# CliMA/LandHydrology.jl

Hardware: AMD Instinct MI355X
Metric: column-cell updates/sec (RHS evals) (higher is better)
Workload: dtype f64

## Files before the change

### landhydrology.jl_amd/csrc/lh_heat_implicit.hpp

```cpp
#pragma once
#include "lh_kernels_impl.hpp"

namespace lh {

template <typename M>
constexpr int heat_implicit_threads() {
    return M::uses_tables ? 512 : 256;
}

template <typename FT>
__device__ __forceinline__ FT heat_boundary_flux(const DevParams<FT>& P, const FaceState<FT>& fs, int face, int64_t col,
                                                 FT T_c) {
    FT fe, fw;
    boundary_fluxes_from<FT, MODEL_HEAT>(P, fs, face, col, T_c, FT(0), FT(0), fe, fw);
    return fe * P.inv_dz;
}

template <typename FT, typename M, bool PERCOL, bool TRBDF2>
__device__ __forceinline__ void heat_implicit_column(const M& mm, DevParams<FT> P, const HeatImplicitArgs<FT>& A,
                                                     int64_t col, FT& nf_acc) {
    const int n = P.nlev;
    const int64_t stride = P.stride;
    const int64_t top = int64_t(n - 1) * stride + col;
    const FT coef = A.coef;
// ... 121 lines not shown
            boundary_constants(kb, kt);
            {
                FT ay = A.al[col] * y[col], be = A.be[col];
                FT Flo = fb_n - Gb * ay;
                forward(kb, kt, [&](int i, int64_t idx) {
                    FT Fhi, ayu = FT(0), beu = FT(0);
                    if (i + 1 < n) {
                        const int64_t idu = idx + stride;
                        ayu = A.al[idu] * y[idu];
                        beu = A.be[idu];
                        Fhi = -A.ks[idx] * (((ayu - ay) + (beu - be)) * P.cg2);
                    } else {
                        Fhi = ft_n + Gt * ay;
                    }
                    const FT f = Flo - Fhi;
                    Flo = Fhi;
                    ay = ayu;
                    be = beu;
                    return y[idx] + coef * f;
                });
            }
            backward([&](int64_t idx, FT x) { z[idx] = (x - c_yn * y[idx]) * c_w2; });
            faces_at(vb1, vt1);
            boundary_constants(kb, kt);
            forward(kb, kt, [&](int, int64_t idx) { return z[idx]; });
            backward(store_y);
        }
    }
}

template <typename FT, typename M, bool PERCOL, bool TRBDF2>
__global__ void __launch_bounds__(heat_implicit_threads<M>())
heat_implicit_kernel(const DevParams<FT> P, const HeatImplicitArgs<FT> A) {
    __shared__ double s_tab[M::uses_tables ? MATH_TAB_DOUBLES : 2];
    const M mm(stage_math_tables<M>(P.math_tab, s_tab));
    const int64_t col = int64_t(blockIdx.x) * blockDim.x + threadIdx.x;
    if (col >= P.ncols) return;
    FT nf_acc = FT(0);
    heat_implicit_column<FT, M, PERCOL, TRBDF2>(mm, P, A, col, nf_acc);
    if (nf_acc != nf_acc) atomicOr(P.status, 1u);
}

template <typename FT>
void launch_heat_implicit(const DevParams<FT>& P, const HeatImplicitArgs<FT>& A, bool percol, bool trbdf2, int math,
                          hipStream_t s) {
    with_math<FT>(math == MATH_LIBM, [&](auto m) { with_bool(percol, [&](auto pc) { with_bool(trbdf2, [&](auto tr) {
        using M = typename decltype(m)::type;
        hipLaunchKernelGGL((heat_implicit_kernel<FT, M, decltype(pc)::value, decltype(tr)::value>),
                           grid_for(P.ncols, heat_implicit_threads<M>()), dim3(heat_implicit_threads<M>()), 0, s, P, A);
    }); }); });
}

#define LH_INSTANTIATE_HEAT_IMPLICIT(FT) \
    template void launch_heat_implicit<FT>(const DevParams<FT>&, const HeatImplicitArgs<FT>&, bool, bool, int, hipStream_t);

}
```

### landhydrology.jl_amd/csrc/lh_implicit.hpp

```cpp
#pragma once
#include "lh_kernels_impl.hpp"

namespace lh {


#define LH_IMPLICIT_DMAX_FRAC 0.5
#define LH_IMPLICIT_STALL 0.9
#define LH_TRBDF2_MAX_STEPS 100000
#define LH_TRBDF2_HMIN_FRAC 1e-10

template <typename FT, bool NOICE>
__device__ __forceinline__ void water_slopes(const ColC<FT>& c, FT vl, FT ti, FT npsi, float& dkr, float& dnpsi) {
    using MF = MathFast<float>;
    dkr = 0.0f;
    dnpsi = 0.0f;
    if (!(vl > c.theta_lim)) return;
    const float num = float(vl - c.theta_r);
    const float m = float(c.m), inv_m = float(c.inv_m);
    const float S = num * float(c.inv_por);
    float w = 0.0f;
    if (S < 1.0f) {
        const float t = MF::exp2(MF::log2(S) * inv_m);
        w = fmaxf(1.0f - t, 1e-7f);
        const float wm = MF::exp2(MF::log2(w) * m);
// ... 16 lines not shown

template <typename FT>
__device__ __forceinline__ FT boundary_flux_slope(const DevParams<FT>& P, const FaceState<FT>& fs, int face,
                                                  FT dK_c, FT dnpsi_c) {
    const int kh = face == FACE_BOTTOM ? P.bc_kind[FACE_BOTTOM][COMP_HYDROLOGY] : P.bc_kind[FACE_TOP][COMP_HYDROLOGY];
    const FT inv_dzb = FT(2) * P.inv_dz;
    if (kh == BC_FREE_DRAINAGE) return -dK_c;
    if (kh == BC_DIRICHLET) {
        return face == FACE_BOTTOM ? fs.K * dnpsi_c * inv_dzb : -fs.K * dnpsi_c * inv_dzb;
    }
    return FT(0);
}

template <typename M>
constexpr int implicit_threads() {
    return M::uses_tables ? 512 : 256;
}

template <typename M>
constexpr bool implicit_variant_exists(bool noice, bool vgf) { return M::is_production || (!noice && !vgf); }

template <typename FT, typename F>
inline void with_implicit_variant(const DevParams<FT>& P, bool percol, bool noice, int math, F&& f) {
    const bool libm = math == MATH_LIBM;
    const bool ni = noice && !libm;
    const bool vg = !libm && !(sizeof(FT) == 8 && P.vg_fast_all == 0);
    with_math<FT>(libm, [&](auto m) { with_bool(percol, [&](auto pc) { with_bool(ni, [&](auto i) { with_bool(vg, [&](auto v) {
        if constexpr (implicit_variant_exists<typename decltype(m)::type>(decltype(i)::value, decltype(v)::value)) f(m, pc, i, v);
    }); }); }); });
}

template <typename M>
__device__ __forceinline__ M implicit_math(const double* math_tab) {
    __shared__ double s_tab[M::uses_tables ? MATH_TAB_DOUBLES : 2];
    return M(stage_math_tables<M>(math_tab, s_tab));
}
__device__ __forceinline__ int64_t implicit_lane_column() { return int64_t(blockIdx.x) * blockDim.x + threadIdx.x; }

template <typename FT, typename M, bool PERCOL, bool NOICE>
struct ColumnSolve {
    static constexpr bool RELK = M::is_production;
    ColC<FT> c;
    FT Ksc, cgw, dmax, floor_r;
    __device__ __forceinline__ ColumnSolve(const M& mm, const DevParams<FT>& P, int64_t col) {
        c = make_colc<FT, M>(P, col, PERCOL);
        if (!NOICE) finish_colc<FT, M>(mm, c);
        Ksc = RELK ? c.Ksat : FT(1);
        cgw = RELK ? c.cgw : P.cg2;
        dmax = FT(LH_IMPLICIT_DMAX_FRAC) * (c.nu - c.theta_r);
        floor_r = c.theta_r;
    }
};

template <typename FT, typename M, bool PERCOL, bool NOICE, bool VGF, bool JAC, typename Row, bool STORE = false>
__device__ __forceinline__ void column_sweep_up(const M& mm, const DevParams<FT>& P,
                                                const ColumnSolve<FT, M, PERCOL, NOICE>& S, const FaceState<FT>& fsb,
                                                const FaceState<FT>& fst, int64_t col, const FT* y, const FT* ti,
                                                FT ti_b, FT coef, FT* cp, FT* dp, Row&& row, FT* sa = nullptr,
                                                FT* sden = nullptr) {
    constexpr bool RELK = ColumnSolve<FT, M, PERCOL, NOICE>::RELK;
    constexpr bool vgf = VGF && M::uses_tables;
    const ColC<FT>& c = S.c;
    const FT Ksc = S.Ksc, cgw = S.cgw;
    const int n = P.nlev;
    const int64_t stride = P.stride;
    const FT T = FT(288);
    auto closures = [&](FT v, FT tiv, FT& K, FT& np, FT& dK, FT& dn) {
// ... 394 lines not shown
```

### landhydrology.jl_amd/csrc/lh_kernels_impl.hpp

```cpp
#pragma once
#include "lh_closures.hpp"
#include "lh_launch.hpp"
#include "lh_dispatch.hpp"
#include "lh_atmos.hpp"
#include <type_traits>

namespace lh {

#ifndef LH_RHS_WAVES_PER_SIMD
#define LH_RHS_WAVES_PER_SIMD 8
#endif
#ifndef LH_RHS_F64_WAVES
#define LH_RHS_F64_WAVES 6
#endif

#ifndef LH_F32C_DT_WAVES
#define LH_F32C_DT_WAVES 5
#endif
#ifndef LH_F32C_DT_VGPRCONST
#define LH_F32C_DT_VGPRCONST 1
#endif
#ifndef LH_F32C_DT_WAVES_SGPR
#define LH_F32C_DT_WAVES_SGPR 8
#endif
// ... 74 lines not shown
    using V = typename Vec<FT, N>::type;
    V v;
    FT* e = reinterpret_cast<FT*>(&v);
#pragma unroll
    for (int j = 0; j < N; ++j) e[j] = in[j];
    if (NT) __builtin_nontemporal_store(v, reinterpret_cast<V*>(p));
    else *reinterpret_cast<V*>(p) = v;
}

template <typename FT, int N, bool NT>
__device__ __forceinline__ void bload(const FT* row, unsigned row_bytes, unsigned lane_byte, FT (&out)[N]) {
    static_assert(sizeof(FT) * N == 8, "one 8-byte access per lane");
    typedef unsigned u32x2 __attribute__((ext_vector_type(2)));
    __amdgpu_buffer_rsrc_t rs = __builtin_amdgcn_make_buffer_rsrc(const_cast<FT*>(row), 0, row_bytes, 0x00020000);
    u32x2 v = __builtin_amdgcn_raw_buffer_load_b64(rs, lane_byte, 0, NT ? 2 : 0);
    __builtin_memcpy(out, &v, 8);
}
template <typename FT, int N, bool NT>
__device__ __forceinline__ void bstore(FT* row, unsigned row_bytes, unsigned lane_byte, const FT (&in)[N]) {
    static_assert(sizeof(FT) * N == 8, "one 8-byte access per lane");
    typedef unsigned u32x2 __attribute__((ext_vector_type(2)));
    __amdgpu_buffer_rsrc_t rs = __builtin_amdgcn_make_buffer_rsrc(row, 0, row_bytes, 0x00020000);
    u32x2 v;
    __builtin_memcpy(&v, in, 8);
    __builtin_amdgcn_raw_buffer_store_b64(v, rs, lane_byte, 0, NT ? 2 : 0);
}

template <int CPL_, int PF_, bool NT_, bool SEG_>
struct KCfg {
    static constexpr int CPL = CPL_, PF = PF_;
    static constexpr bool NT = NT_, SEG = SEG_;
};

template <typename M>
__device__ __forceinline__ MathTables stage_math_tables(const double* gtab, double* lds) {
    MathTables t;
    t.log_tab = lds;
    t.exp_tab = lds + 2 * LOG_TAB_N;
    if (M::uses_tables) {
        for (int i = threadIdx.x; i < MATH_TAB_DOUBLES; i += blockDim.x) lds[i] = gtab[i];
        __syncthreads();
    }
    return t;
}

template <typename FT> struct Bits;
template <> struct Bits<double> { using type = unsigned long long; };
template <> struct Bits<float> { using type = unsigned int; };

__device__ __forceinline__ double fmax_ft(double a, double b) { return __builtin_fmax(a, b); }
__device__ __forceinline__ float fmax_ft(float a, float b) { return __builtin_fmaxf(a, b); }
__device__ __forceinline__ double fmin_ft(double a, double b) { return __builtin_fmin(a, b); }
__device__ __forceinline__ float fmin_ft(float a, float b) { return __builtin_fminf(a, b); }

__device__ __forceinline__ float max_nonneg(float a, float b) {
    return __builtin_bit_cast(float, __builtin_elementwise_max(__builtin_bit_cast(int, a), __builtin_bit_cast(int, b)));
}

__device__ __forceinline__ void wave_sync() {
    __builtin_amdgcn_fence(__ATOMIC_RELEASE, "wavefront");
    __builtin_amdgcn_wave_barrier();
    __builtin_amdgcn_fence(__ATOMIC_ACQUIRE, "wavefront");
}

template <typename FT>
__device__ __forceinline__ bool finite(FT x) {
    return x - x == FT(0);
}

template <typename M>
constexpr bool noice_exists(bool factors) { return M::is_production && !factors; }
template <typename M, int MODEL>
constexpr bool robust_vg_exists() { return M::uses_tables && MODEL != MODEL_HEAT; }
// ... 16 lines not shown
    constexpr bool WATER = (MODEL != MODEL_HEAT);
    constexpr bool HEAT = (MODEL != MODEL_RICHARDS);
    constexpr bool TEND_MODE = (MODE == 0 || MODE == 4);
    DevParams<FT> P = P0;
    if constexpr (heat_vgpr_constants<FT, MODEL, FACTORS, PERCOL, M, NOICE>() && TEND_MODE && (!FACTORS || PERCOL || MODE == 4)) {
        auto vr = [](FT& x) { asm volatile("" : "+v"(x)); };
        vr(P.rho_c_ds); vr(P.rhocp_l); vr(P.rhocp_i); vr(P.T_ref); vr(P.kappa_sat_unfrozen);
        vr(P.l2_kappa_sat_unfrozen); vr(P.l2_kappa_sat_frozen); vr(P.kersten_exp_unfrozen);
        vr(P.kersten_exp_frozen); vr(P.neg_b_log2e_sc);
        if (MODE != 4) {
            vr(P.rho_i); vr(P.LH_f0); vr(P.inv_dz); vr(P.half_inv_dz);
            if (FACTORS) { vr(P.gamma); vr(P.T_ref_visc); vr(P.Omega); }
        }
    }
#ifndef LH_F64_FACTORS_PARTIAL_PIN
#define LH_F64_FACTORS_PARTIAL_PIN 3
#endif
#ifndef LH_F64_FACTORS_PARTIAL_PIN_STAGES
#define LH_F64_FACTORS_PARTIAL_PIN_STAGES 0
#endif
    if constexpr (LH_F64_FACTORS_PARTIAL_PIN > 0 && heat_vgpr_constants<FT, MODEL, FACTORS, PERCOL, M, NOICE>() &&
                  (MODE == 0 || (LH_F64_FACTORS_PARTIAL_PIN_STAGES && MODE != 4)) &&
                  FACTORS && !PERCOL) {
        auto vr = [](FT& x) { asm volatile("" : "+v"(x)); };
        vr(P.rho_c_ds); vr(P.rhocp_l); vr(P.T_ref);
        if (LH_F64_FACTORS_PARTIAL_PIN >= 5) { vr(P.rhocp_i); vr(P.rho_i); }
        if (LH_F64_FACTORS_PARTIAL_PIN >= 8) { vr(P.LH_f0); vr(P.gamma); vr(P.Omega); }
    }
    constexpr int CPL = CFG::CPL, PF = CFG::PF;
    constexpr bool NT = CFG::NT;
    constexpr bool TEND = (MODE == 0 || MODE == 4);
    constexpr bool WANT_DT = (MODE == 4);
    const FT dt = (!TEND && dt_device) ? *dt_device : dt_value;
    __shared__ double s_tab[M::uses_tables ? MATH_TAB_DOUBLES : 2];
    extern __shared__ __align__(16) unsigned char s_dyn[];
    const int n = P.nlev;
    float* s_red = reinterpret_cast<float*>(s_dyn);
    if (WANT_DT) s_red[threadIdx.x] = 0.0f;
    __shared__ unsigned s_waves_done;
    if (WANT_DT && threadIdx.x == 0) s_waves_done = 0u;
    constexpr bool MAY_PROF = (MODEL == MODEL_HEAT) || (MODEL == MODEL_RICHARDS && FACTORS);
    FT* s_pf = reinterpret_cast<FT*>(s_dyn + (WANT_DT ? ((size_t(blockDim.x) * sizeof(float) + 15) & ~size_t(15)) : 0));
    const FT* pf_T = (MAY_PROF && MODEL == MODEL_RICHARDS) ? P.aux_prof[3] : nullptr;
    const FT* pf_vl = (MAY_PROF && MODEL == MODEL_HEAT) ? P.aux_prof[0] : nullptr;
    const FT* pf_ti = (MAY_PROF && MODEL == MODEL_HEAT) ? P.aux_prof[1] : nullptr;
    if constexpr (MAY_PROF) {
        for (int i = threadIdx.x; i < n; i += blockDim.x) {
            if (pf_T) s_pf[i] = pf_T[i];
            if (pf_vl) s_pf[i] = pf_vl[i];
            if (pf_ti) s_pf[n + i] = pf_ti[i];
        }
    }
    const M mm(stage_math_tables<M>(P.math_tab, s_tab));
    if (!M::uses_tables) __syncthreads();

    unsigned blk = blockIdx.x;
    if (P.xcd_remap) {
        const unsigned per = gridDim.x >> 3;
        if (blk < (per << 3)) blk = (blk & 7u) * per + (blk >> 3);
    }
    const int64_t col0 = (int64_t(blk) * blockDim.x + threadIdx.x) * CPL;
    if (col0 >= P.ncols) return;
    const int64_t stride = P.stride;
    constexpr bool SEG = CFG::SEG;
    const int i_lo = SEG ? int(blockIdx.y) * P.seg_len : 0;
    const int i_hi = SEG ? (i_lo + P.seg_len < n ? i_lo + P.seg_len : n) : n;
    const int i_first = (SEG && i_lo > 0) ? i_lo - 1 : 0;
    const int i_end = (SEG && i_hi < n) ? i_hi + 1 : n;
    const unsigned lane_byte = (unsigned)col0 * (unsigned)sizeof(FT);
    const unsigned row_bytes = (unsigned)(stride * (int64_t)sizeof(FT));
    constexpr bool BUF = (sizeof(FT) * CPL == 8);
    auto rload = [&](const FT* row, FT (&out)[CPL]) {
        if constexpr (BUF) bload<FT, CPL, NT>(row, row_bytes, lane_byte, out);
        else vload<FT, CPL, NT>(row + col0, out);
    };
    auto rstore = [&](FT* row, const FT (&in)[CPL]) {
        if constexpr (BUF) bstore<FT, CPL, NT>(row, row_bytes, lane_byte, in);
        else vstore<FT, CPL, NT>(row + col0, in);
    };

    const int64_t in0 = SEG ? stride * i_first : 0, out0 = SEG ? stride * i_lo : 0;
    constexpr bool FROM_K1 = (MODE == 5);
    const FT* r_vl = (MODEL == MODEL_HEAT ? AUX.v[0] : (FROM_K1 ? BASE.v[0] : IN.v[0])) + in0;
    const FT* r_ti = NOICE ? nullptr : (MODEL == MODEL_HEAT ? AUX.v[1] : (TEND ? IN.v[1] : BASE.v[1])) + in0;
    const FT* r_re = HEAT ? (FROM_K1 ? BASE.v[2] : IN.v[2]) + in0 : nullptr;
    const FT* r_k1v = (FROM_K1 && WATER) ? IN.v[0] + in0 : nullptr;
    const FT* r_k1e = (FROM_K1 && HEAT) ? IN.v[2] + in0 : nullptr;
    const bool need_Taux = (MODEL == MODEL_RICHARDS) && FACTORS && P.viscosity_kind;
    const FT* r_Ta = need_Taux ? AUX.v[3] + in0 : nullptr;
    const FT* b_vl = ((MODE == 2 || MODE == 3) && WATER) ? BASE.v[0] + out0 : nullptr;
    const FT* b_re = ((MODE == 2 || MODE == 3) && HEAT) ? BASE.v[2] + out0 : nullptr;
    FT* o_vl = WATER ? OUT.v[0] + out0 : nullptr;
    FT* o_re = HEAT ? OUT.v[2] + out0 : nullptr;

    ColC<FT> c[CPL];
    int64_t colj[CPL];
#pragma unroll
    for (int j = 0; j < CPL; ++j) {
        colj[j] = col0 + j < P.ncols ? col0 + j : P.ncols - 1;
        c[j] = make_colc<FT, M>(P, colj[j], PERCOL);
        if (WATER && !NOICE) finish_colc<FT, M>(mm, c[j]);
        if constexpr (M::uses_tables && WATER && !PERCOL && !HEAT) asm volatile("" : "+v"(c[j].e_log2_alpha));
    }
    if constexpr (f32_coupled_vgpr_constants<FT, MODEL, FACTORS, PERCOL, M, MODE>()) {
        auto vr = [](FT& x) { asm volatile("" : "+v"(x)); };
        ColC<FT>& q = c[0];
        vr(q.nu); vr(q.theta_lim); vr(q.theta_r); vr(q.inv_por); vr(q.e_inv_m); vr(q.e_m); vr(q.e_one);
        vr(q.e_inv_n); vr(q.e_log2_alpha); vr(q.Ksat); vr(q.inv_S_s); vr(q.inv_nu); vr(q.k_dry);
        if (!NOICE) vr(q.l2_por);
#pragma unroll
        for (int j = 1; j < CPL; ++j) c[j] = c[0];
    }

    constexpr bool vgf = VGF && M::uses_tables;
    constexpr bool RELK = M::is_production;
    const FT cgT = P.cg2;
    FT cgw[CPL], Ksc[CPL];
#pragma unroll
    for (int j = 0; j < CPL; ++j) {
        Ksc[j] = RELK ? c[j].Ksat : FT(1);
        cgw[j] = RELK ? c[j].cgw : cgT;
    }

    FT vl[CPL], ti[CPL], re[CPL], Ta[CPL];
    FT vl_n[PF][CPL], ti_n[PF][CPL], re_n[PF][CPL], Ta_n[PF][CPL];
    FT kv_n[PF][CPL], ke_n[PF][CPL];
    FT vl_p[CPL], re_p[CPL];
    FT yv[CPL], ye[CPL], yv_p[CPL], ye_p[CPL];
    FT K_p[CPL], psi_p[CPL], T_p[CPL], kap_p[CPL], E_p[CPL];
    FT Fw_lo[CPL], Fe_lo[CPL];
    FT nf_acc = FT(0);
    float dpsi_p[CPL], ircs_p[CPL], DmaxW[CPL], DmaxT[CPL];
    float DmaxWb[CPL];

#pragma unroll
    for (int j = 0; j < CPL; ++j) {
        K_p[j] = psi_p[j] = T_p[j] = kap_p[j] = E_p[j] = Fw_lo[j] = Fe_lo[j] = FT(0);
        vl_p[j] = re_p[j] = FT(0);
        yv[j] = ye[j] = yv_p[j] = ye_p[j] = FT(0);
        vl[j] = ti[j] = re[j] = FT(0);
        Ta[j] = FT(288);
        dpsi_p[j] = DmaxW[j] = DmaxWb[j] = DmaxT[j] = ircs_p[j] = 0.0f;
    }
    int lev_f = i_first;
    auto fetch = [&](int slot) {
        if (MAY_PROF && pf_vl) {
#pragma unroll
            for (int j = 0; j < CPL; ++j) vl_n[slot][j] = s_pf[lev_f];
        } else rload(r_vl, vl_n[slot]);
        if (!NOICE) {
            if (MAY_PROF && pf_ti) {
#pragma unroll
                for (int j = 0; j < CPL; ++j) ti_n[slot][j] = s_pf[n + lev_f];
            } else rload(r_ti, ti_n[slot]);
        }
        if (HEAT) rload(r_re, re_n[slot]);
        if (need_Taux) {
            if (MAY_PROF && pf_T) {
#pragma unroll
                for (int j = 0; j < CPL; ++j) Ta_n[slot][j] = s_pf[lev_f];
            } else rload(r_Ta, Ta_n[slot]);
        }
        ++lev_f;
        if (FROM_K1 && WATER) { rload(r_k1v, kv_n[slot]); r_k1v += stride; }
        if (FROM_K1 && HEAT) { rload(r_k1e, ke_n[slot]); r_k1e += stride; }
        r_vl += stride;
        if (!NOICE) r_ti += stride;
        if (HEAT) r_re += stride;
        if (need_Taux) r_Ta += stride;
    };
#pragma unroll
    for (int k = 0; k < PF; ++k) {
#pragma unroll
        for (int j = 0; j < CPL; ++j) {
            vl_n[k][j] = ti_n[k][j] = re_n[k][j] = kv_n[k][j] = ke_n[k][j] = FT(0);
            Ta_n[k][j] = FT(288);
        }
        if (i_first + k < i_end) fetch(k);
    }

    auto emit = [&](const FT (&Fw_hi)[CPL], const FT (&Fe_hi)[CPL], const FT (&u_vl)[CPL],
                    const FT (&u_re)[CPL], const FT (&y_vl)[CPL], const FT (&y_re)[CPL]) {
        FT dvl[CPL], dre[CPL];
#pragma unroll
        for (int j = 0; j < CPL; ++j) {
            dvl[j] = WATER ? Fw_lo[j] - Fw_hi[j] : FT(0);
            dre[j] = HEAT ? Fe_lo[j] - Fe_hi[j] : FT(0);
            if (CPL == 1 || col0 + j < P.ncols) {
                if (WATER) nf_acc = fma_ft(dvl[j], FT(0), nf_acc);
                if (HEAT) nf_acc = fma_ft(dre[j], FT(0), nf_acc);
            }
        }
        if (TEND) {
            if (WATER) rstore(o_vl, dvl);
            if (HEAT) rstore(o_re, dre);
        } else {
            auto stage = [&](const FT* brow, FT* orow, const FT (&u)[CPL], const FT (&k)[CPL], const FT (&yb)[CPL]) {
                FT b[CPL], r[CPL];
                if (MODE == 2 || MODE == 3) rload(brow, b);
#pragma unroll
                for (int j = 0; j < CPL; ++j) {
                    if (FROM_K1) b[j] = yb[j];
                    if (MODE == 1)
                        r[j] = u[j] + dt * k[j];
                    else if (MODE == 2 || MODE == 5)
                        r[j] = (FT(3) * b[j] + u[j] + dt * k[j]) * FT(0.25);
                    else {
                        const FT sum = b[j] + FT(2) * u[j] + FT(2) * dt * k[j];
                        const FT q = sum * FT(1.0 / 3.0);
                        r[j] = fma_ft(fma_ft(FT(-3), q, sum), FT(1.0 / 3.0), q);
                    }
// ... 4 lines not shown
            if (HEAT) stage(b_re, o_re, u_re, dre, y_re);
        }
        if (WATER) {
            o_vl += stride;
            if (MODE == 2 || MODE == 3) b_vl += stride;
        }
        if (HEAT) {
            o_re += stride;
            if (MODE == 2 || MODE == 3) b_re += stride;
        }
    };

#if LH_RHS_OUTER_UNROLL > 0
#pragma unroll RHS_OUTER_UNROLL
#endif
    for (int i0 = i_first; i0 < i_end; i0 += PF) {
#pragma unroll
      for (int k = 0; k < PF; ++k) {
        const int i = i0 + k;
        if (PF > 1 && i >= i_end) break;
#pragma unroll
        for (int j = 0; j < CPL; ++j) {
            vl[j] = vl_n[k][j];
            ti[j] = NOICE ? FT(0) : ti_n[k][j];
            re[j] = re_n[k][j];
            Ta[j] = Ta_n[k][j];
            if (FROM_K1) {
                yv[j] = vl[j];
                ye[j] = re[j];
                if (WATER) vl[j] = yv[j] + dt * kv_n[k][j];
                if (HEAT) re[j] = ye[j] + dt * ke_n[k][j];
            }
        }
        if (i + PF < i_end) fetch(k);
        FT K[CPL], psi[CPL], T[CPL], kap[CPL], E[CPL], rcs[CPL];
        float dpsi[CPL], ircs[CPL];
#pragma unroll
        for (int j = 0; j < CPL; ++j) {
            T[j] = Ta[j];
            kap[j] = FT(0);
            K[j] = psi[j] = E[j] = FT(0);
            dpsi[j] = ircs[j] = 0.0f;
            rcs[j] = FT(1);
            if (HEAT) {
                T[j] = temperature_closure<FT, M, NOICE>(mm, P, c[j], vl[j], ti[j], re[j], rcs[j]);
                kap[j] = kappa_closure<FT, M, NOICE>(mm, P, c[j], vl[j], ti[j]);
                if (WANT_DT) ircs[j] = float(mm.rcp(rcs[j]));
            }
            if (WATER) {
                water_closures<FT, M, FACTORS, true, WANT_DT, NOICE, RELK, HEAT, true>(mm, P, c[j], vl[j], ti[j], T[j], K[j],
                                                                                       psi[j], &dpsi[j], vgf);
                if (HEAT) E[j] = (P.rhocp_l * (T[j] - P.T_ref)) * K[j];
            }
            if (WANT_DT && i > i_first) {
                if (WATER) DmaxW[j] = max_nonneg(DmaxW[j], float(K_p[j] + K[j]) * max_nonneg(dpsi_p[j], dpsi[j]));
                if (HEAT) DmaxT[j] = max_nonneg(DmaxT[j], float(kap_p[j] + kap[j]) * max_nonneg(ircs_p[j], ircs[j]));
            }
        }
        if (i == 0) {
#pragma unroll
            for (int j = 0; j < CPL; ++j) {
                FT K_f = FT(0), kap_f = FT(0);
                const FT K_c = K[j] * Ksc[j];
                boundary_fluxes<FT, M, MODEL, FACTORS, NOICE>(mm, P, c[j], FACE_BOTTOM, colj[j], vl[j], ti[j],
                                                              T[j], K_c, -psi[j], Fe_lo[j], Fw_lo[j], &K_f, &kap_f, vgf);
                Fe_lo[j] = Fe_lo[j] * P.inv_dz;
                Fw_lo[j] = Fw_lo[j] * P.inv_dz;
// ... 1 lines not shown
                    DmaxW[j] = max_nonneg(DmaxW[j], 2.0f * float(K[j]) * dpsi[j]);
                    DmaxWb[j] = max_nonneg(DmaxWb[j], 4.0f * float(fmax_ft(K_f, K_f > FT(0) ? K_c : FT(0))) * dpsi[j]);
                    if (HEAT) {
                        DmaxT[j] = max_nonneg(DmaxT[j], 2.0f * float(kap[j]) * ircs[j]);
                        DmaxT[j] = max_nonneg(DmaxT[j], 4.0f * float(fmax_ft(kap_f, kap_f > FT(0) ? kap[j] : FT(0))) * ircs[j]);
                    }
                }
            }
        } else if (!SEG || i > i_first) {
            FT Fw[CPL], Fe[CPL];
#pragma unroll
            for (int j = 0; j < CPL; ++j) {
                Fw[j] = Fe[j] = FT(0);
                FT gh = FT(0);
                if (WATER) {
                    gh = head_difference(psi[j], psi_p[j], P.dz) * cgw[j];
                    Fw[j] = -(K_p[j] + K[j]) * gh;
                }
                if (HEAT) {
                    FT gT = (T[j] - T_p[j]) * cgT;
                    Fe[j] = -(kap_p[j] + kap[j]) * gT;
                    if (WATER) Fe[j] = Fe[j] - (E_p[j] + E[j]) * gh;
                }
            }
            if (!SEG || i > i_lo) emit(Fw, Fe, vl_p, re_p, yv_p, ye_p);
#pragma unroll
            for (int j = 0; j < CPL; ++j) {
                Fw_lo[j] = Fw[j];
                Fe_lo[j] = Fe[j];
            }
        }
#pragma unroll
        for (int j = 0; j < CPL; ++j) {
            vl_p[j] = vl[j];
            re_p[j] = re[j];
            if (FROM_K1) {
                yv_p[j] = yv[j];
                ye_p[j] = ye[j];
            }
            K_p[j] = K[j];
            psi_p[j] = psi[j];
            T_p[j] = T[j];
            kap_p[j] = kap[j];
            E_p[j] = E[j];
            if (WANT_DT) {
                dpsi_p[j] = dpsi[j];
                ircs_p[j] = ircs[j];
            }
        }
      }
    }
    if (!SEG || i_hi == n) {
        FT Fw[CPL], Fe[CPL];
#pragma unroll
        for (int j = 0; j < CPL; ++j) {
            FT K_f = FT(0), kap_f = FT(0);
            const FT K_c = K_p[j] * Ksc[j];
            boundary_fluxes<FT, M, MODEL, FACTORS, NOICE>(mm, P, c[j], FACE_TOP, colj[j], vl[j], ti[j], T_p[j],
                                                          K_c, -psi_p[j], Fe[j], Fw[j], &K_f, &kap_f, vgf);
            Fe[j] = Fe[j] * P.inv_dz;
            Fw[j] = Fw[j] * P.inv_dz;
            if (WANT_DT) {
                DmaxW[j] = max_nonneg(DmaxW[j], 2.0f * float(K_p[j]) * dpsi_p[j]);
                DmaxWb[j] = max_nonneg(DmaxWb[j], 4.0f * float(fmax_ft(K_f, K_f > FT(0) ? K_c : FT(0))) * dpsi_p[j]);
                if (HEAT) {
                    DmaxT[j] = max_nonneg(DmaxT[j], 2.0f * float(kap_p[j]) * ircs_p[j]);
                    DmaxT[j] = max_nonneg(DmaxT[j], 4.0f * float(fmax_ft(kap_f, kap_f > FT(0) ? kap_p[j] : FT(0))) * ircs_p[j]);
                }
            }
        }
        emit(Fw, Fe, vl_p, re_p, yv_p, ye_p);
    }
    if (nf_acc != nf_acc) atomicOr(P.status, 1u);
    if (WANT_DT) {
        using U = typename Bits<FT>::type;
        float dmax = 0.0f;
#pragma unroll
        for (int j = 0; j < CPL; ++j) {
// ... 18 lines not shown
            const unsigned nw = lanes_left >= int64_t(blockDim.x) ? nwaves : unsigned((lanes_left + 63) >> 6);
            if (atomicAdd(&s_waves_done, 1u) == nw - 1u) {
                for (unsigned w = 0; w < nwaves; ++w) dmax = max_nonneg(dmax, s_red[w << 6]);
                if (dmax > 0.0f) {
                    const FT best = (FT(2) * dt * P.dz * P.dz) / FT(dmax);
                    U b;
                    __builtin_memcpy(&b, &best, sizeof(FT));
                    U* word = reinterpret_cast<U*>(P.dt_out);
                    if (b < __atomic_load_n(word, __ATOMIC_RELAXED)) atomicMin(word, b);
                }
            }
        }
    }
}

constexpr int CS_FACE_WORDS = 8;
template <int MODEL> constexpr int cs_exchange_arrays() {
    return MODEL == MODEL_COUPLED ? 5 : 2;
}
template <int MODEL> constexpr int cs_flux_arrays() {
    return MODEL == MODEL_COUPLED ? 2 : 1;
}
static inline int cs_fetch_tiles(int model, bool noice, bool need_Taux) {
    if (model == MODEL_RICHARDS) return 1 + (noice ? 0 : 1) + (need_Taux ? 2 : 0);
    return 3;
}

template <typename FT, int MODEL, bool FACTORS, bool PERCOL, typename M, bool NOICE = false, bool VGF = true>
__global__ void __launch_bounds__(1024)
column_stepper_kernel(const DevParams<FT> P0, const Planes<FT> Y, const Planes<FT> AUX, const FT dt_value,
                      const FT* __restrict__ dt_device, const int64_t nsteps, const FT* __restrict__ bcv) {
    constexpr bool WATER = (MODEL != MODEL_HEAT);
    constexpr bool HEAT = (MODEL != MODEL_RICHARDS);
    __shared__ double s_tab[M::uses_tables ? MATH_TAB_DOUBLES : 2];
    extern __shared__ __align__(16) unsigned char s_dyn[];
    const int n = P0.nlev;
    const int tpc = (n + 63) & ~63;
    const int slot = int(threadIdx.x) / tpc;
    const int cpb = int(blockDim.x) / tpc;
    const FT dt = dt_device ? *dt_device : dt_value;
    constexpr int NARR = cs_exchange_arrays<MODEL>();
    FT* sK = reinterpret_cast<FT*>(s_dyn) + size_t(slot) * NARR * n;
    FT* sh = sK + n;
    FT* sT = WATER ? sh + n : sK;
    FT* sKap = sT + n;
    FT* sE = sKap + n;
    const M mm(stage_math_tables<M>(P0.math_tab, s_tab));
    if (!M::uses_tables) __syncthreads();
    DevParams<FT> P = P0;
    const int i = int(threadIdx.x) - slot * tpc;
    unsigned blk = blockIdx.x;
    if (P.xcd_remap) {
        const unsigned per = gridDim.x >> 3;
        if (blk < (per << 3)) blk = (blk & 7u) * per + (blk >> 3);
    }
    const int64_t col_raw = int64_t(blk) * cpb + slot;
    const bool cell = i < n && col_raw < P.ncols;
    const int ic = i < n ? i : n - 1;
    const int64_t col = col_raw < P.ncols ? col_raw : P.ncols - 1;
    ColC<FT> c = make_colc<FT, M>(P, col, PERCOL);
    if (WATER && !NOICE) finish_colc<FT, M>(mm, c);
    constexpr bool vgf = VGF && M::uses_tables;
    constexpr bool RELK = M::is_production;
    const FT cgT = P.cg2;
    const FT Ksc = RELK ? c.Ksat : FT(1);
    const FT cgw = RELK ? c.cgw : cgT;
    const bool need_Taux = (MODEL == MODEL_RICHARDS) && FACTORS && P.viscosity_kind;
// ... 125 lines not shown
        if (col_first + cs < P.ncols) {
            const int64_t g = int64_t(lev) * P.stride + col_first + cs;
            if (WATER) Y.v[0][g] = tiles[cs * n + lev];
            if (HEAT) Y.v[2][g] = tiles[tile_n + cs * n + lev];
        }
    }
    if (cell && nf_acc != nf_acc) atomicOr(P.status, 1u);
}

template <typename T>
__device__ __forceinline__ T wave_uniform(const T& x) {
    static_assert(sizeof(T) % 4 == 0, "32-bit words");
    uint32_t w[sizeof(T) / 4];
    __builtin_memcpy(w, &x, sizeof(T));
#pragma unroll
    for (size_t k = 0; k < sizeof(T) / 4; ++k) w[k] = __builtin_amdgcn_readfirstlane(w[k]);
    T r;
    __builtin_memcpy(&r, w, sizeof(T));
    return r;
}

template <typename FT, int MODEL, bool FACTORS, bool PERCOL, typename M, int CW, bool NOICE>
constexpr int cs_wave_min_waves() {
    if (!M::uses_tables || MODEL != MODEL_RICHARDS) return 4;
    if (CW == 1) return 6;
    return (NOICE && !FACTORS) ? 6 : 4;
}
template <typename FT, int MODEL, bool FACTORS, bool PERCOL, typename M, int CW, bool NOICE = false, bool VGF = true, bool BOUND = false>
__global__ void __launch_bounds__(1024, (cs_wave_min_waves<FT, MODEL, FACTORS, PERCOL, M, CW, NOICE>()))
column_stepper_wave_kernel(const DevParams<FT> P0, const Planes<FT> Y, const Planes<FT> AUX, const FT dt_value,
                           const FT* __restrict__ dt_device, const int64_t nsteps, const FT* __restrict__ bcv) {
    constexpr bool WATER = (MODEL != MODEL_HEAT);
    constexpr bool HEAT = (MODEL != MODEL_RICHARDS);
    __shared__ double s_tab[M::uses_tables ? MATH_TAB_DOUBLES : 2];
    extern __shared__ __align__(16) unsigned char s_dyn[];
    const int n = P0.nlev;
    const int slot = int(threadIdx.x) >> 6;
    const int l = int(threadIdx.x) & 63;
    const int cpb = int(blockDim.x) >> 6;
    const FT dt = dt_device ? *dt_device : dt_value;
    constexpr int NEX = cs_exchange_arrays<MODEL>();
    constexpr int NARR = NEX + cs_flux_arrays<MODEL>();
    constexpr size_t COLW = size_t(NARR) * 64 + CS_FACE_WORDS;
    FT* sK = reinterpret_cast<FT*>(s_dyn) + size_t(slot) * COLW;
    FT* sh = sK + 64;
    FT* sT = WATER ? sh + 64 : sK;
    FT* sKap = sT + 64;
    FT* sE = sKap + 64;
    FT* sFw = sK + size_t(NEX) * 64;
    FT* sFe = WATER ? sFw + 64 : sFw;
    FT* sFace = sK + size_t(NARR) * 64;
    const M mm(stage_math_tables<M>(P0.math_tab, s_tab));
    if (!M::uses_tables) __syncthreads();
    DevParams<FT> P = P0;
    unsigned blk = blockIdx.x;
    if (P.xcd_remap) {
        const unsigned per = gridDim.x >> 3;
        if (blk < (per << 3)) blk = (blk & 7u) * per + (blk >> 3);
    }
    const int64_t col_raw = int64_t(blk) * cpb + slot;
    const int64_t col = col_raw < P.ncols ? col_raw : P.ncols - 1;
    ColC<FT> c = make_colc<FT, M>(P, col, PERCOL);
    if (WATER && !NOICE) finish_colc<FT, M>(mm, c);
    if constexpr (PERCOL) c = wave_uniform(c);
    constexpr bool vgf = VGF && M::uses_tables;
    constexpr bool RELK = M::is_production;
    const FT cgT = P.cg2;
// ... 267 lines not shown
                U b;
                __builtin_memcpy(&b, &best, sizeof(FT));
                U* word = reinterpret_cast<U*>(P.dt_out);
                if (b < __atomic_load_n(word, __ATOMIC_RELAXED)) atomicMin(word, b);
            }
        }
    }
    __syncthreads();
#pragma unroll
    for (int q = 0; q < CW; ++q) {
        const int i = CW * l + q;
        if (i < n) {
            if (WATER) tiles[slot * n + i] = y_vl[q];
            if (HEAT) tiles[tile_n + slot * n + i] = y_re[q];
        }
    }
    __syncthreads();
    for (int e = threadIdx.x; e < tile_n; e += blockDim.x) {
        const int lev = e / cpb, cs = e - lev * cpb;
        if (col_first + cs < P.ncols) {
            const int64_t g = int64_t(lev) * P.stride + col_first + cs;
            if (WATER) Y.v[0][g] = tiles[cs * n + lev];
            if (HEAT) Y.v[2][g] = tiles[tile_n + cs * n + lev];
        }
    }
    if (col_raw < P.ncols && nf_acc != nf_acc) atomicOr(P.status, 1u);
}

template <typename FT, int MODEL, bool FACTORS, bool PERCOL, typename M>
__global__ void __launch_bounds__(256)
diag_kernel(const DevParams<FT> P, const Planes<FT> IN, const Planes<FT> AUX, const Planes<FT> OUT) {
    constexpr bool WATER = (MODEL != MODEL_HEAT);
    constexpr bool HEAT = (MODEL != MODEL_RICHARDS);
    __shared__ double s_tab[M::uses_tables ? MATH_TAB_DOUBLES : 1];
    const M mm(stage_math_tables<M>(P.math_tab, s_tab));
    const int64_t col = int64_t(blockIdx.x) * blockDim.x + threadIdx.x;
    if (col >= P.ncols) return;
    const FT* p_vl = (MODEL == MODEL_HEAT ? AUX.v[0] : IN.v[0]) + col;
    const FT* p_ti = (MODEL == MODEL_HEAT ? AUX.v[1] : IN.v[1]) + col;
    const bool need_Taux = (MODEL == MODEL_RICHARDS) && FACTORS && P.viscosity_kind;
    ColC<FT> c = make_colc<FT, M>(P, col, PERCOL);
    if (WATER) finish_colc<FT, M>(mm, c);
    const bool vgf = M::uses_tables && P.vg_fast_all != 0;
    for (int i = 0; i < P.nlev; ++i) {
        const int64_t o = int64_t(i) * P.stride;
        FT vl = p_vl[o], ti = p_ti[o];
        FT T = need_Taux ? AUX.v[3][o + col] : FT(288), kap = FT(0), K = FT(0), psi = FT(0);
        if (HEAT) {
            FT rcs;
            T = temperature_closure<FT, M>(mm, P, c, vl, ti, IN.v[2][o + col], rcs);
            kap = kappa_closure<FT, M>(mm, P, c, vl, ti);
        }
        if (WATER) water_closures<FT, M, FACTORS>(mm, P, c, vl, ti, T, K, psi, nullptr, vgf);
        OUT.v[0][o + col] = K;
        OUT.v[1][o + col] = psi;
        OUT.v[2][o + col] = kap;
        OUT.v[3][o + col] = T;
    }
}

template <typename FT, int MODEL, bool FACTORS, bool PERCOL, typename M>
__global__ void __launch_bounds__(256)
boundary_flux_kernel(const DevParams<FT> P, const Planes<FT> IN, const Planes<FT> AUX, const int face, FT* out_e, FT* out_w) {
    constexpr bool WATER = (MODEL != MODEL_HEAT);
    constexpr bool HEAT = (MODEL != MODEL_RICHARDS);
    __shared__ double s_tab[M::uses_tables ? MATH_TAB_DOUBLES : 1];
    const M mm(stage_math_tables<M>(P.math_tab, s_tab));
    const int64_t col = int64_t(blockIdx.x) * blockDim.x + threadIdx.x;
    if (col >= P.ncols) return;
    const int64_t o = int64_t(face == FACE_BOTTOM ? 0 : P.nlev - 1) * P.stride + col;
    ColC<FT> c = make_colc<FT, M>(P, col, PERCOL);
    if (WATER) finish_colc<FT, M>(mm, c);
    const bool vgf = M::uses_tables && P.vg_fast_all != 0;
    const bool need_Taux = (MODEL == MODEL_RICHARDS) && FACTORS && P.viscosity_kind;
    const FT vl = (MODEL == MODEL_HEAT ? AUX.v[0] : IN.v[0])[o];
    const FT ti = (MODEL == MODEL_HEAT ? AUX.v[1] : IN.v[1])[o];
    FT T = need_Taux ? AUX.v[3][o] : FT(288), K = FT(0), psi = FT(0), rcs = FT(1);
    if (HEAT) T = temperature_closure<FT, M>(mm, P, c, vl, ti, IN.v[2][o], rcs);
    constexpr bool RELK = M::is_production;
    if (WATER) {
        water_closures<FT, M, FACTORS, true, false, false, RELK>(mm, P, c, vl, ti, T, K, psi, nullptr, vgf);
        if (RELK) K = K * c.Ksat;
    }
    FT fe, fw;
    boundary_fluxes<FT, M, MODEL, FACTORS, false>(mm, P, c, face, col, vl, ti, T, K, psi, fe, fw, nullptr, nullptr, vgf);
    if (P.bc_kind[face][COMP_ENERGY] == BC_NONE) fe = FT(NAN);
    if (P.bc_kind[face][COMP_HYDROLOGY] == BC_NONE) fw = FT(NAN);
    out_e[col] = fe;
    out_w[col] = fw;
}


template <typename FT, int MODEL, bool PERCOL, typename M>
__global__ void __launch_bounds__(256)
stable_dt_kernel(const DevParams<FT> P, const Planes<FT> IN, const Planes<FT> AUX, const FT courant,
                 typename Bits<FT>::type* out_bits) {
    constexpr bool WATER = (MODEL != MODEL_HEAT);
    constexpr bool HEAT = (MODEL != MODEL_RICHARDS);
    using U = typename Bits<FT>::type;
    __shared__ double s_tab[M::uses_tables ? MATH_TAB_DOUBLES : 1];
    const M mm(stage_math_tables<M>(P.math_tab, s_tab));
    const int64_t col = int64_t(blockIdx.x) * blockDim.x + threadIdx.x;
    FT best = FT(INFINITY);
    if (col < P.ncols) {
        const FT* p_vl = (MODEL == MODEL_HEAT ? AUX.v[0] : IN.v[0]) + col;
        const FT* p_ti = (MODEL == MODEL_HEAT ? AUX.v[1] : IN.v[1]) + col;
        ColC<FT> c = make_colc<FT, M>(P, col, PERCOL);
        if (WATER) finish_colc<FT, M>(mm, c);
        const FT cdz2 = courant * P.dz * P.dz;
        const int n = P.nlev;
        FT K_p = FT(0), dpsi_p = FT(0), kap_p = FT(0), rcs_p = FT(1);
        for (int i = 0; i < n; ++i) {
            const int64_t o = int64_t(i) * P.stride;
            FT vl = p_vl[o], ti = p_ti[o];
            FT K = FT(0), dpsi = FT(0), kap = FT(0), rcs = FT(1);
            FT Tc = FT(288);
            if (MODEL == MODEL_RICHARDS && P.viscosity_kind) Tc = AUX.v[3][o + col];
            if (HEAT) Tc = temperature_closure<FT, M>(mm, P, c, vl, ti, IN.v[2][o + col], rcs);
            if (WATER) {
                FT psi;
                water_closures<FT, M, true>(mm, P, c, vl, ti, Tc, K, psi);
                const FT nu_eff = c.nu - ti;
                const FT vls = !(vl <= c.theta_lim) ? vl : c.theta_lim;
                const FT Se = (vls - c.theta_r) / (nu_eff - c.theta_r);
                const FT u = mm.pow(Se, -c.inv_m) - FT(1);
                if (Se <= FT(1) && u > FT(0))
                    dpsi = fabs(psi) * (u + FT(1)) / (c.n * c.m * u * Se * (nu_eff - c.theta_r));
                else
                    dpsi = FT(1) / c.S_s;
            }
            if (HEAT) kap = kappa_closure<FT, M>(mm, P, c, vl, ti);
            FT D = FT(0);
            if (i == 0 || i == n - 1) {
// ... 490 lines not shown
```

Measured before the change: 286.6 billion.

## Overlap first-level prefetch with math table staging and vectorize table copy

Moves the initial prefetch of the first PF levels ahead of the shared-memory math table staging, so global loads for column data are in flight while the LDS tables are copied and synchronized; dead lanes now participate in the barrier and return afterwards. The table staging copy is rewritten to use 16-byte paired loads batched six deep, with an empty asm barrier forcing all loads to issue before stores, and the shared arrays get 16-byte alignment to allow this. It also restricts the per-level carry-over of previous-cell values to the variables each model actually uses. The cost is higher register pressure from holding prefetch buffers across the staging phase, which could reduce occupancy.

Measured after the change: 289.0 billion, median of 6. About the same (+0.8%).

```diff
diff --git a/landhydrology.jl_amd/csrc/lh_heat_implicit.hpp b/landhydrology.jl_amd/csrc/lh_heat_implicit.hpp
--- a/landhydrology.jl_amd/csrc/lh_heat_implicit.hpp
+++ b/landhydrology.jl_amd/csrc/lh_heat_implicit.hpp
@@ -177,7 +177,7 @@
 template <typename FT, typename M, bool PERCOL, bool TRBDF2>
 __global__ void __launch_bounds__(heat_implicit_threads<M>())
 heat_implicit_kernel(const DevParams<FT> P, const HeatImplicitArgs<FT> A) {
-    __shared__ double s_tab[M::uses_tables ? MATH_TAB_DOUBLES : 2];
+    __shared__ __align__(16) double s_tab[M::uses_tables ? MATH_TAB_DOUBLES : 2];
     const M mm(stage_math_tables<M>(P.math_tab, s_tab));
     const int64_t col = int64_t(blockIdx.x) * blockDim.x + threadIdx.x;
     if (col >= P.ncols) return;
diff --git a/landhydrology.jl_amd/csrc/lh_implicit.hpp b/landhydrology.jl_amd/csrc/lh_implicit.hpp
--- a/landhydrology.jl_amd/csrc/lh_implicit.hpp
+++ b/landhydrology.jl_amd/csrc/lh_implicit.hpp
@@ -72,7 +72,7 @@
 
 template <typename M>
 __device__ __forceinline__ M implicit_math(const double* math_tab) {
-    __shared__ double s_tab[M::uses_tables ? MATH_TAB_DOUBLES : 2];
+    __shared__ __align__(16) double s_tab[M::uses_tables ? MATH_TAB_DOUBLES : 2];
     return M(stage_math_tables<M>(math_tab, s_tab));
 }
 __device__ __forceinline__ int64_t implicit_lane_column() { return int64_t(blockIdx.x) * blockDim.x + threadIdx.x; }
diff --git a/landhydrology.jl_amd/csrc/lh_kernels_impl.hpp b/landhydrology.jl_amd/csrc/lh_kernels_impl.hpp
--- a/landhydrology.jl_amd/csrc/lh_kernels_impl.hpp
+++ b/landhydrology.jl_amd/csrc/lh_kernels_impl.hpp
@@ -130,13 +130,34 @@
     static constexpr bool NT = NT_, SEG = SEG_;
 };
 
+constexpr int MATH_TAB_BATCH = 6;
 template <typename M>
 __device__ __forceinline__ MathTables stage_math_tables(const double* gtab, double* lds) {
     MathTables t;
     t.log_tab = lds;
     t.exp_tab = lds + 2 * LOG_TAB_N;
     if (M::uses_tables) {
-        for (int i = threadIdx.x; i < MATH_TAB_DOUBLES; i += blockDim.x) lds[i] = gtab[i];
+        typedef double d2 __attribute__((ext_vector_type(2)));
+        static_assert(MATH_TAB_DOUBLES % 2 == 0, "the tables are staged in pairs");
+        constexpr int PAIRS = MATH_TAB_DOUBLES / 2;
+        const d2* g2 = reinterpret_cast<const d2*>(gtab);
+        d2* l2 = reinterpret_cast<d2*>(lds);
+        const int step = int(blockDim.x);
+        for (int i0 = int(threadIdx.x); i0 < PAIRS; i0 += MATH_TAB_BATCH * step) {
+            d2 v[MATH_TAB_BATCH];
+#pragma unroll
+            for (int k = 0; k < MATH_TAB_BATCH; ++k) {
+                const int i = i0 + k * step;
+                v[k] = g2[i < PAIRS ? i : PAIRS - 1];
+            }
+#pragma unroll
+            for (int k = 0; k < MATH_TAB_BATCH; ++k) asm volatile("" : "+v"(v[k]));
+#pragma unroll
+            for (int k = 0; k < MATH_TAB_BATCH; ++k) {
+                const int i = i0 + k * step;
+                if (i < PAIRS) l2[i] = v[k];
+            }
+        }
         __syncthreads();
     }
     return t;
@@ -219,7 +240,7 @@
     constexpr bool TEND = (MODE == 0 || MODE == 4);
     constexpr bool WANT_DT = (MODE == 4);
     const FT dt = (!TEND && dt_device) ? *dt_device : dt_value;
-    __shared__ double s_tab[M::uses_tables ? MATH_TAB_DOUBLES : 2];
+    __shared__ __align__(16) double s_tab[M::uses_tables ? MATH_TAB_DOUBLES : 2];
     extern __shared__ __align__(16) unsigned char s_dyn[];
     const int n = P.nlev;
     float* s_red = reinterpret_cast<float*>(s_dyn);
@@ -238,8 +259,6 @@
             if (pf_ti) s_pf[n + i] = pf_ti[i];
         }
     }
-    const M mm(stage_math_tables<M>(P.math_tab, s_tab));
-    if (!M::uses_tables) __syncthreads();
 
     unsigned blk = blockIdx.x;
     if (P.xcd_remap) {
@@ -247,7 +266,7 @@
         if (blk < (per << 3)) blk = (blk & 7u) * per + (blk >> 3);
     }
     const int64_t col0 = (int64_t(blk) * blockDim.x + threadIdx.x) * CPL;
-    if (col0 >= P.ncols) return;
+    const bool live = col0 < P.ncols;
     const int64_t stride = P.stride;
     constexpr bool SEG = CFG::SEG;
     const int i_lo = SEG ? int(blockIdx.y) * P.seg_len : 0;
@@ -261,6 +280,9 @@
         if constexpr (BUF) bload<FT, CPL, NT>(row, row_bytes, lane_byte, out);
         else vload<FT, CPL, NT>(row + col0, out);
     };
+    auto rload_if = [&](bool on, const FT* row, FT (&out)[CPL]) {
+        if (on) rload(row, out);
+    };
     auto rstore = [&](FT* row, const FT (&in)[CPL]) {
         if constexpr (BUF) bstore<FT, CPL, NT>(row, row_bytes, lane_byte, in);
         else vstore<FT, CPL, NT>(row + col0, in);
@@ -280,6 +302,51 @@
     FT* o_vl = WATER ? OUT.v[0] + out0 : nullptr;
     FT* o_re = HEAT ? OUT.v[2] + out0 : nullptr;
 
+    FT vl_n[PF][CPL], ti_n[PF][CPL], re_n[PF][CPL], Ta_n[PF][CPL];
+    FT kv_n[PF][CPL], ke_n[PF][CPL];
+    int lev_f = i_first;
+    auto fetch = [&](int slot, auto early) {
+        constexpr bool EARLY = decltype(early)::value;
+        const bool on = EARLY ? live : true;
+        if (MAY_PROF && pf_vl) {
+#pragma unroll
+            for (int j = 0; j < CPL; ++j) vl_n[slot][j] = EARLY ? pf_vl[lev_f] : s_pf[lev_f];
+        } else rload_if(on, r_vl, vl_n[slot]);
+        if (!NOICE) {
+            if (MAY_PROF && pf_ti) {
+#pragma unroll
+                for (int j = 0; j < CPL; ++j) ti_n[slot][j] = EARLY ? pf_ti[lev_f] : s_pf[n + lev_f];
+            } else rload_if(on, r_ti, ti_n[slot]);
+        }
+        if (HEAT) rload_if(on, r_re, re_n[slot]);
+        if (need_Taux) {
+            if (MAY_PROF && pf_T) {
+#pragma unroll
+                for (int j = 0; j < CPL; ++j) Ta_n[slot][j] = EARLY ? pf_T[lev_f] : s_pf[lev_f];
+            } else rload_if(on, r_Ta, Ta_n[slot]);
+        }
+        ++lev_f;
+        if (FROM_K1 && WATER) { rload_if(on, r_k1v, kv_n[slot]); r_k1v += stride; }
+        if (FROM_K1 && HEAT) { rload_if(on, r_k1e, ke_n[slot]); r_k1e += stride; }
+        r_vl += stride;
+        if (!NOICE) r_ti += stride;
+        if (HEAT) r_re += stride;
+        if (need_Taux) r_Ta += stride;
+    };
+#pragma unroll
+    for (int k = 0; k < PF; ++k) {
+#pragma unroll
+        for (int j = 0; j < CPL; ++j) {
+            vl_n[k][j] = ti_n[k][j] = re_n[k][j] = kv_n[k][j] = ke_n[k][j] = FT(0);
+            Ta_n[k][j] = FT(288);
+        }
+        if (i_first + k < i_end) fetch(k, std::true_type{});
+    }
+
+    const M mm(stage_math_tables<M>(P.math_tab, s_tab));
+    if (!M::uses_tables) __syncthreads();
+    if (!live) return;
+
     ColC<FT> c[CPL];
     int64_t colj[CPL];
 #pragma unroll
@@ -310,8 +377,6 @@
     }
 
     FT vl[CPL], ti[CPL], re[CPL], Ta[CPL];
-    FT vl_n[PF][CPL], ti_n[PF][CPL], re_n[PF][CPL], Ta_n[PF][CPL];
-    FT kv_n[PF][CPL], ke_n[PF][CPL];
     FT vl_p[CPL], re_p[CPL];
     FT yv[CPL], ye[CPL], yv_p[CPL], ye_p[CPL];
     FT K_p[CPL], psi_p[CPL], T_p[CPL], kap_p[CPL], E_p[CPL];
@@ -328,42 +393,6 @@
         vl[j] = ti[j] = re[j] = FT(0);
         Ta[j] = FT(288);
         dpsi_p[j] = DmaxW[j] = DmaxWb[j] = DmaxT[j] = ircs_p[j] = 0.0f;
-    }
-    int lev_f = i_first;
-    auto fetch = [&](int slot) {
-        if (MAY_PROF && pf_vl) {
-#pragma unroll
-            for (int j = 0; j < CPL; ++j) vl_n[slot][j] = s_pf[lev_f];
-        } else rload(r_vl, vl_n[slot]);
-        if (!NOICE) {
-            if (MAY_PROF && pf_ti) {
-#pragma unroll
-                for (int j = 0; j < CPL; ++j) ti_n[slot][j] = s_pf[n + lev_f];
-            } else rload(r_ti, ti_n[slot]);
-        }
-        if (HEAT) rload(r_re, re_n[slot]);
-        if (need_Taux) {
-            if (MAY_PROF && pf_T) {
-#pragma unroll
-                for (int j = 0; j < CPL; ++j) Ta_n[slot][j] = s_pf[lev_f];
-            } else rload(r_Ta, Ta_n[slot]);
-        }
-        ++lev_f;
-        if (FROM_K1 && WATER) { rload(r_k1v, kv_n[slot]); r_k1v += stride; }
-        if (FROM_K1 && HEAT) { rload(r_k1e, ke_n[slot]); r_k1e += stride; }
-        r_vl += stride;
-        if (!NOICE) r_ti += stride;
-        if (HEAT) r_re += stride;
-        if (need_Taux) r_Ta += stride;
-    };
-#pragma unroll
-    for (int k = 0; k < PF; ++k) {
-#pragma unroll
-        for (int j = 0; j < CPL; ++j) {
-            vl_n[k][j] = ti_n[k][j] = re_n[k][j] = kv_n[k][j] = ke_n[k][j] = FT(0);
-            Ta_n[k][j] = FT(288);
-        }
-        if (i_first + k < i_end) fetch(k);
     }
 
     auto emit = [&](const FT (&Fw_hi)[CPL], const FT (&Fe_hi)[CPL], const FT (&u_vl)[CPL],
@@ -434,7 +463,7 @@
                 if (HEAT) re[j] = ye[j] + dt * ke_n[k][j];
             }
         }
-        if (i + PF < i_end) fetch(k);
+        if (i + PF < i_end) fetch(k, std::false_type{});
         FT K[CPL], psi[CPL], T[CPL], kap[CPL], E[CPL], rcs[CPL];
         float dpsi[CPL], ircs[CPL];
 #pragma unroll
@@ -502,18 +531,22 @@
         }
 #pragma unroll
         for (int j = 0; j < CPL; ++j) {
-            vl_p[j] = vl[j];
-            re_p[j] = re[j];
-            if (FROM_K1) {
+            if constexpr (!TEND) {
+                if constexpr (WATER) vl_p[j] = vl[j];
+                if constexpr (HEAT) re_p[j] = re[j];
+            }
+            if constexpr (FROM_K1) {
                 yv_p[j] = yv[j];
                 ye_p[j] = ye[j];
             }
-            K_p[j] = K[j];
-            psi_p[j] = psi[j];
+            if constexpr (WATER) {
+                K_p[j] = K[j];
+                psi_p[j] = psi[j];
+            }
             T_p[j] = T[j];
-            kap_p[j] = kap[j];
-            E_p[j] = E[j];
-            if (WANT_DT) {
+            if constexpr (HEAT) kap_p[j] = kap[j];
+            if constexpr (HEAT && WATER) E_p[j] = E[j];
+            if constexpr (WANT_DT) {
                 dpsi_p[j] = dpsi[j];
                 ircs_p[j] = ircs[j];
             }
@@ -598,7 +631,7 @@
                       const FT* __restrict__ dt_device, const int64_t nsteps, const FT* __restrict__ bcv) {
     constexpr bool WATER = (MODEL != MODEL_HEAT);
     constexpr bool HEAT = (MODEL != MODEL_RICHARDS);
-    __shared__ double s_tab[M::uses_tables ? MATH_TAB_DOUBLES : 2];
+    __shared__ __align__(16) double s_tab[M::uses_tables ? MATH_TAB_DOUBLES : 2];
     extern __shared__ __align__(16) unsigned char s_dyn[];
     const int n = P0.nlev;
     const int tpc = (n + 63) & ~63;
@@ -790,7 +823,7 @@
                            const FT* __restrict__ dt_device, const int64_t nsteps, const FT* __restrict__ bcv) {
     constexpr bool WATER = (MODEL != MODEL_HEAT);
     constexpr bool HEAT = (MODEL != MODEL_RICHARDS);
-    __shared__ double s_tab[M::uses_tables ? MATH_TAB_DOUBLES : 2];
+    __shared__ __align__(16) double s_tab[M::uses_tables ? MATH_TAB_DOUBLES : 2];
     extern __shared__ __align__(16) unsigned char s_dyn[];
     const int n = P0.nlev;
     const int slot = int(threadIdx.x) >> 6;
@@ -1124,7 +1157,7 @@
 diag_kernel(const DevParams<FT> P, const Planes<FT> IN, const Planes<FT> AUX, const Planes<FT> OUT) {
     constexpr bool WATER = (MODEL != MODEL_HEAT);
     constexpr bool HEAT = (MODEL != MODEL_RICHARDS);
-    __shared__ double s_tab[M::uses_tables ? MATH_TAB_DOUBLES : 1];
+    __shared__ __align__(16) double s_tab[M::uses_tables ? MATH_TAB_DOUBLES : 1];
     const M mm(stage_math_tables<M>(P.math_tab, s_tab));
     const int64_t col = int64_t(blockIdx.x) * blockDim.x + threadIdx.x;
     if (col >= P.ncols) return;
@@ -1156,7 +1189,7 @@
 boundary_flux_kernel(const DevParams<FT> P, const Planes<FT> IN, const Planes<FT> AUX, const int face, FT* out_e, FT* out_w) {
     constexpr bool WATER = (MODEL != MODEL_HEAT);
     constexpr bool HEAT = (MODEL != MODEL_RICHARDS);
-    __shared__ double s_tab[M::uses_tables ? MATH_TAB_DOUBLES : 1];
+    __shared__ __align__(16) double s_tab[M::uses_tables ? MATH_TAB_DOUBLES : 1];
     const M mm(stage_math_tables<M>(P.math_tab, s_tab));
     const int64_t col = int64_t(blockIdx.x) * blockDim.x + threadIdx.x;
     if (col >= P.ncols) return;
@@ -1190,7 +1223,7 @@
     constexpr bool WATER = (MODEL != MODEL_HEAT);
     constexpr bool HEAT = (MODEL != MODEL_RICHARDS);
     using U = typename Bits<FT>::type;
-    __shared__ double s_tab[M::uses_tables ? MATH_TAB_DOUBLES : 1];
+    __shared__ __align__(16) double s_tab[M::uses_tables ? MATH_TAB_DOUBLES : 1];
     const M mm(stage_math_tables<M>(P.math_tab, s_tab));
     const int64_t col = int64_t(blockIdx.x) * blockDim.x + threadIdx.x;
     FT best = FT(INFINITY);
```
